# tennisonliu/bayesian-neural-network

Hardware: AMD Instinct MI355X
Metric: MC-forward-samples/sec + KL-elements/sec, 784-1200-1200-10 BNN (higher is better)
Workload: dtype bf16

## Files before the change

### bayesian-neural-network_amd/csrc/bbb_linear.hip

```cpp
#include "bnn_device.h"
#include "bnn_fin.h"
#include "bbb_sample_body.h"
#include "bbb_block_gemm.h"
#include "../../include/bnn_hip.h"
#include <string.h>

namespace bnn {

struct BbbK {
  const void* x;
  long x_sstride;
  const float* w_mu;
  const float* w_rho;
  const float* w_sigma;
  const float* b_mu;
  const float* b_rho;
  const float* eps_w;
  const float* eps_b;
  float* eps_w_dump;
  float* eps_b_dump;
  void* y;
  float4* ws;
  int S, B, K, N;
  __bf16* y16;
// ... 175 lines not shown
        bf16x4 o;
#pragma unroll
        for (int i = 0; i < 4; ++i) o[i] = (__bf16)v[i];
        *reinterpret_cast<bf16x4*>(yp) = o;
      } else {
#pragma unroll
        for (int i = 0; i < 4; ++i)
          if (nb + i < N) yp[i] = (__bf16)v[i];
      }
      if (p.y_lo) {
        __bf16* lp = reinterpret_cast<__bf16*>(p.y_lo) + yoff;
        bf16x4 l;
#pragma unroll
        for (int i = 0; i < 4; ++i) l[i] = (__bf16)(v[i] - (float)(__bf16)v[i]);
        if (vec_ok) {
          *reinterpret_cast<bf16x4*>(lp) = l;
        } else {
#pragma unroll
          for (int i = 0; i < 4; ++i)
            if (nb + i < N) lp[i] = l[i];
        }
      }
    } else {
      float* yp = reinterpret_cast<float*>(p.y) + yoff;
      if (vec_ok) {
        *reinterpret_cast<float4*>(yp) = make_float4(v[0], v[1], v[2], v[3]);
      } else {
#pragma unroll
        for (int i = 0; i < 4; ++i)
          if (nb + i < N) yp[i] = v[i];
      }
      if (p.y16) {
        __bf16* cp = p.y16 + yoff;
        if (vec_ok) {
          bf16x4 o;
#pragma unroll
          for (int i = 0; i < 4; ++i) o[i] = (__bf16)v[i];
          *reinterpret_cast<bf16x4*>(cp) = o;
        } else {
#pragma unroll
          for (int i = 0; i < 4; ++i)
            if (nb + i < N) cp[i] = (__bf16)v[i];
        }
      }
    }
  }
}

struct FinPack : FinTail {
  int ks;
  uint32_t* ks_ticket;
  float4* ks_stats;
  float* ks_tiles;
};

template <int MATH, int XDT, int R, bool ALIGNED, bool FINAL, bool TRANS = false, bool PRE = false, int MT = 8, bool WT = false,
          bool XTL = false>
__device__ __forceinline__ bool bbb_fwd_body(const BbbK& p, const FinPack* fp) {
  constexpr int F = 16 / R;
  static_assert(!XTL || (FINAL && R == 1 && ALIGNED && MT == 8 && XDT == BNN_BF16 && MATH == BNN_MATH_BF16),
                "piece-order x: the fused output layer in bf16 math");
  extern __shared__ __attribute__((aligned(16))) float lds[];
  const int lane = threadIdx.x & 63, wave = threadIdx.x >> 6, nw = blockDim.x >> 6;
  const int r = lane & 15, q = lane >> 4;
  const int c = r / F, f = r % F;
  const int K = p.K, N = p.N, B = p.B;
  const int ntiles = (N + F - 1) / F, mbs = (B + 16 * MT - 1) / (16 * MT);
  int item;
  const int KS = FINAL ? fp->ks : 1;
  if (!xcd_work_item(ntiles * p.S * mbs * KS, item)) return false;
  const int ks = item % KS;
  item /= KS;
  const int nt = item / (p.S * mbs), s = (item / mbs) % p.S, mb = item % mbs;
  const int n = nt * F + f;
  const bool n_ok = n < N;
  const int nc = min(n, N - 1);
  const int m0 = mb * (16 * MT);
  const int mtiles = min(MT, (B - m0 + 15) >> 4);
  const int ssteps = (K + 32 * R - 1) / (32 * R);
  const int spb = (ssteps + KS - 1) / KS;
  const int t_lo = ks * spb, t_hi = min(ssteps, t_lo + spb);
  const uint32_t gs = global_sample(p, s);
  const bool do_stats = p.want_stats && mb == 0;
  const bool do_ls = do_stats && (s == 0 || FINAL);
  const bool do_dump = mb == 0;
  const int gpr = (int)eps_groups_per_row(K);
  const uint32_t wid = eps_tensor_id(p.layer_id, kEpsWeight);
  const char* xs = reinterpret_cast<const char*>(p.x) + (size_t)(s / p.xg) * (size_t)p.x_sstride * (XDT == BNN_F32 ? 4 : 2);
  constexpr bool X3 = MATH == BNN_MATH_BF16X3;
  static_assert(!X3 || (!TRANS && !PRE && !WT), "the split-bf16 mode is a forward sampling form");
  const char* xs_lo = (X3 && XDT == BNN_BF16) ? reinterpret_cast<const char*>(p.x_lo) + (size_t)(s / p.xg) * (size_t)p.x_sstride * 2 : nullptr;

  float* lds_bias = lds + (size_t)nw * MT * 64 * 4;
  float* lds_red = lds_bias + 16;
  f32x4* slab = reinterpret_cast<f32x4*>(lds);

  BNN_STAMP(0);
  BNN_STAMP_RT(8);
  f32x4 acc[MT];
#pragma unroll
  for (int m = 0; m < MT; ++m) acc[m] = f32x4{0.f, 0.f, 0.f, 0.f};
  float s_e2 = 0.f, s_a = 0.f, s_ls = 0.f;
  if (do_stats && item == 0 && ks == 0 && threadIdx.x == 0)
    p.ws[0] = make_float4(__int_as_float(ntiles), 0.f, 0.f, 0.f);

  float mu_n[8], rho_n[8];
  float4 wraw_n = make_float4(0.f, 0.f, 0.f, 0.f);
  auto load_params = [&](int t) {
    const int k = (t * R + c) * 32 + q * 8;
    if (PRE && TRANS) {
      bf16x8 tw;
#pragma unroll
      for (int j = 0; j < 8; ++j) {
        const __bf16 v = p.w_pre[((size_t)s * K + min(k + j, K - 1)) * p.ldw + nc];
        tw[j] = (k + j < K && n_ok) ? v : (__bf16)0.f;
      }
      wraw_n = __builtin_bit_cast(float4, tw);
    } else if (PRE) {
      wraw_n = *reinterpret_cast<const float4*>(p.w_pre + ((size_t)s * N + nc) * K + min(k, K - 8));
    } else if (TRANS) {
#pragma unroll
      for (int j = 0; j < 8; ++j) {
        const size_t woff = (size_t)min(k + j, K - 1) * p.ldw + nc;
        mu_n[j] = p.w_mu[woff];
        rho_n[j] = p.w_rho[woff];
      }
    } else if (ALIGNED) {
      const size_t woff = (size_t)nc * K + min(k, K - 8);
      load8<true>(p.w_mu + woff, 8, mu_n);
      load8<true>(p.w_rho + woff, 8, rho_n);
    } else {
      const int valid = n_ok ? min(8, K - k) : 0;
      const size_t woff = (size_t)n * K + k;
      load8<false>(p.w_mu + woff, valid, mu_n);
      load8<false>(p.w_rho + woff, valid, rho_n);
    }
  };
  if (t_lo + wave < t_hi) load_params(t_lo + wave);
  float bmu_pre = 0.f, brho_pre = 0.f, beps_pre = 0.f;
  if (PRE) {
    if (!TRANS && wave == nw - 1 && lane < F && n_ok && ks == 0 && p.b_pre) bmu_pre = p.b_pre[(size_t)s * N + n];
  } else if (!TRANS && wave == nw - 1 && lane < F && n_ok && ks == 0) {
    bmu_pre = p.b_mu[n];
    brho_pre = p.b_rho[n];
    beps_pre = bias_eps(p, n, s, gs, do_dump);
  }

#pragma nounroll
  for (int t = t_lo + wave; t < t_hi; t += nw) {
    const int k = (t * R + c) * 32 + q * 8;
    const int valid = n_ok ? min(8, K - k) : 0;
    constexpr int FR = (XDT == BNN_F32 || X3) ? 2 : 1;
    constexpr int MC0 = (8 / (R * FR)) < 1 ? 1 : (8 / (R * FR));
    constexpr int MC = MC0 > MT ? MT : MC0;
    float4 xraw[MC * R * FR];
    auto stage = [&](int ch) {
#pragma unroll
      for (int mm = 0; mm < MC; ++mm) {
        if constexpr (XTL) {
          xraw[mm] = *reinterpret_cast<const float4*>(xs + ((size_t)((t * 8 + ch * MC + mm) * 64 + lane)) * 16);
          continue;
        }
        const int row = m0 + (ch * MC + mm) * 16 + r;
#pragma unroll
        for (int cc = 0; cc < R; ++cc) {
          const int xk = (t * R + cc) * 32 + q * 8;
          if (ALIGNED) {
            const size_t off = (size_t)min(row, B - 1) * K + min(xk, K - 8);
            if (XDT == BNN_F32) {
              const float4* px = reinterpret_cast<const float4*>(reinterpret_cast<const float*>(xs) + off);
              xraw[(mm * R + cc) * 2 + 0] = px[0];
              xraw[(mm * R + cc) * 2 + 1] = px[1];
            } else if (X3) {
              xraw[(mm * R + cc) * 2 + 0] = *reinterpret_cast<const float4*>(reinterpret_cast<const __bf16*>(xs) + off);
              xraw[(mm * R + cc) * 2 + 1] = *reinterpret_cast<const float4*>(reinterpret_cast<const __bf16*>(xs_lo) + off);
            } else {
              xraw[mm * R + cc] = *reinterpret_cast<const float4*>(reinterpret_cast<const __bf16*>(xs) + off);
            }
          } else {
            const int xvalid = (row < B) ? min(8, K - xk) : 0;
            const size_t off = (size_t)row * K + xk;
            if (XDT == BNN_F32) {
              float v[8];
              load8<false>(reinterpret_cast<const float*>(xs) + off, xvalid, v);
              xraw[(mm * R + cc) * 2 + 0] = make_float4(v[0], v[1], v[2], v[3]);
              xraw[(mm * R + cc) * 2 + 1] = make_float4(v[4], v[5], v[6], v[7]);
            } else {
              bf16x8 vb;
#pragma unroll
              for (int j = 0; j < 8; ++j)
                vb[j] = (j < xvalid) ? (reinterpret_cast<const __bf16*>(xs) + off)[j] : (__bf16)0.0f;
              if (X3) {
                bf16x8 vl;
#pragma unroll
                for (int j = 0; j < 8; ++j)
                  vl[j] = (j < xvalid) ? (reinterpret_cast<const __bf16*>(xs_lo) + off)[j] : (__bf16)0.0f;
                xraw[(mm * R + cc) * 2 + 0] = __builtin_bit_cast(float4, vb);
                xraw[(mm * R + cc) * 2 + 1] = __builtin_bit_cast(float4, vl);
              } else {
// ... 129 lines not shown
              bf16x8 xb;
              if (XDT == BNN_F32) {
                const float4 lo = xraw[(mm * R + cc) * 2], hi = xraw[(mm * R + cc) * 2 + 1];
                xb[0] = (__bf16)lo.x; xb[1] = (__bf16)lo.y; xb[2] = (__bf16)lo.z; xb[3] = (__bf16)lo.w;
                xb[4] = (__bf16)hi.x; xb[5] = (__bf16)hi.y; xb[6] = (__bf16)hi.z; xb[7] = (__bf16)hi.w;
              } else {
                xb = __builtin_bit_cast(bf16x8, xraw[mm * R + cc]);
              }
              acc[m] = __builtin_amdgcn_mfma_f32_16x16x32_bf16((R == 1 || c == cc) ? wa : wz, xb, acc[m], 0, 0, 0);
            } else {
              float xv[8];
              if (XDT == BNN_F32) {
                const float4 lo = xraw[(mm * R + cc) * 2], hi = xraw[(mm * R + cc) * 2 + 1];
                xv[0] = lo.x; xv[1] = lo.y; xv[2] = lo.z; xv[3] = lo.w;
                xv[4] = hi.x; xv[5] = hi.y; xv[6] = hi.z; xv[7] = hi.w;
              } else {
                const bf16x8 xb = __builtin_bit_cast(bf16x8, xraw[mm * R + cc]);
#pragma unroll
                for (int j = 0; j < 8; ++j) xv[j] = (float)xb[j];
              }
#pragma unroll
              for (int j = 0; j < 8; ++j)
                acc[m] = __builtin_amdgcn_mfma_f32_16x16x4f32((R == 1 || c == cc) ? w[j] : 0.f, xv[j], acc[m], 0, 0, 0);
            }
          }
        }
        if ((ch + 1) * MC < MT && (ch + 1) * MC < mtiles) stage(ch + 1);
      }
    }
  }

  asm volatile("" :: "v"(acc[0][0]), "v"(acc[MT - 1][3]));
  BNN_STAMP(3);
  if (wave == nw - 1 && lane < 16) {
    float b = 0.f;
    if (PRE) b = (!TRANS && lane < F && n_ok && ks == 0) ? bmu_pre : 0.f;
    else if (!TRANS && lane < F && n_ok && ks == 0) b = sample_bias(p, bmu_pre, brho_pre, beps_pre, do_stats, do_ls, s_e2, s_a, s_ls);
    lds_bias[lane] = b;
  }
#pragma unroll
  for (int m = 0; m < MT; ++m)
    if (m < mtiles) slab[(wave * MT + m) * 64 + lane] = acc[m];
  if (do_stats) {
    const float a = wave_sum(s_e2), b = wave_sum(s_a), cc = wave_sum(s_ls);
    if (lane == 0) {
      lds_red[wave * 3 + 0] = a;
      lds_red[wave * 3 + 1] = b;
      lds_red[wave * 3 + 2] = cc;
    }
  }
  BNN_STAMP(4);
  __syncthreads();
  BNN_STAMP(5);
  float own0 = 0.f, own1 = 0.f, own2 = 0.f;
  if (do_stats && threadIdx.x == 0) {
    for (int wv = 0; wv < nw; ++wv) {
      own0 += lds_red[wv * 3 + 0];
      own1 += lds_red[wv * 3 + 1];
      own2 += lds_red[wv * 3 + 2];
    }
    if (KS == 1) p.ws[1 + (size_t)s * ntiles + nt] = make_float4(own0, own1, own2, 0.f);
  }
  float* fin_lg = lds_red + 3 * nw;
  if (!FINAL || KS == 1) {
    epilogue_store<R, MT>(p, slab, lds_bias, nw, mtiles, nt, s, m0, FINAL ? fin_lg : nullptr);
  }
  BNN_STAMP(6);
  BNN_STAMP_RT(9);
  if (FINAL) {
    const FinK& fk = fp->k;
    float* part = reinterpret_cast<float*>((reinterpret_cast<uintptr_t>(fin_lg + 128 * 16) + 7) & ~(uintptr_t)7);
    int T[8];
#pragma unroll
    for (int l = 0; l < 8; ++l)
      T[l] = (l < fk.n_layers - 1) ? __float_as_int(reinterpret_cast<const float4*>(fk.ws[l])[0].x) : 0;
    if (KS > 1) {
      float* mine = fp->ks_tiles + ((size_t)s * KS + ks) * (128 * 16);
      epilogue_store<R>(p, slab, lds_bias, nw, 8, nt, s, m0, nullptr, mine);
      if (threadIdx.x == 0) fp->ks_stats[(size_t)s * KS + ks] = make_float4(own0, own1, own2, 0.f);
      asm volatile("s_waitcnt vmcnt(0)" ::: "memory");
      __syncthreads();
      uint32_t* flag = reinterpret_cast<uint32_t*>(part);
      if (threadIdx.x == 0) {
        __builtin_amdgcn_fence(__ATOMIC_RELEASE, "agent");
        asm volatile("s_waitcnt vmcnt(0)" ::: "memory");
        const uint32_t tk = __hip_atomic_fetch_add(fp->ks_ticket + s, 1u, __ATOMIC_RELAXED, __HIP_MEMORY_SCOPE_AGENT);
        const uint32_t last = (tk == (uint32_t)KS - 1u) ? 1u : 0u;
        if (last) {
          __builtin_amdgcn_fence(__ATOMIC_ACQUIRE, "agent");
          asm volatile("s_waitcnt vmcnt(0)" ::: "memory");
        }
        *flag = last;
      }
      __syncthreads();
      BNN_STAMP(7);
      if (*flag == 0u) return true;
      __syncthreads();
      const float* tiles = fp->ks_tiles + (size_t)s * KS * (128 * 16);
      float4 q4 = make_float4(0.f, 0.f, 0.f, 0.f);
      if ((int)threadIdx.x < KS) q4 = fp->ks_stats[(size_t)s * KS + threadIdx.x];
      for (int it = threadIdx.x; it < 128 * 4; it += blockDim.x) {
        const int brow = it >> 2, fg = it & 3;
        f32x4 v = f32x4{0.f, 0.f, 0.f, 0.f};
        for (int j = 0; j < KS; ++j) v += *reinterpret_cast<const f32x4*>(tiles + (size_t)j * (128 * 16) + brow * 16 + fg * 4);
        if (p.relu) {
#pragma unroll
          for (int i = 0; i < 4; ++i) v[i] = fmaxf(v[i], 0.f);
        }
        *reinterpret_cast<f32x4*>(fin_lg + brow * 16 + fg * 4) = v;
        if (brow < B) {
          float* yp = reinterpret_cast<float*>(p.y) + ((size_t)s * B + brow) * N + fg * 4;
#pragma unroll
          for (int i = 0; i < 4; ++i)
            if (fg * 4 + i < N) yp[i] = v[i];
        }
      }
      if (threadIdx.x < 64) {
        own0 = wave_sum(q4.x);
        own1 = wave_sum(q4.y);
        own2 = wave_sum(q4.z);
      }
      if (threadIdx.x == 0) {
        p.ws[1 + (size_t)s * ntiles + nt] = make_float4(own0, own1, own2, 0.f);
        fp->ks_ticket[s] = 0u;
      }
    }
    __syncthreads();
    BNN_STAMP(10);
    float a = 0.f, b = 0.f, nll = 0.f;
    const int own_layer = fk.n_layers - 1;
#ifdef BNN_STAMPS
    fin_sample(fk, fp->c, s, T, fin_lg, 16, own_layer, own0, own1, own2, part, a, b, nll, p.dbg ? p.dbg + (size_t)blockIdx.x * 16 : nullptr);
#else
    fin_sample(fk, fp->c, s, T, fin_lg, 16, own_layer, own0, own1, own2, part, a, b, nll);
#endif
    BNN_STAMP(11);
    if (threadIdx.x == 0) {
      fin_store(fk, s, a, b, nll);
      if (fk.S == 1) {
        if (fp->sums) {
          float* so = fp->sums;
          so[0] = a; so[1] = b; so[2] = nll; so[3] = 1.f;
        }
        if (fk.sample_counter) *fk.sample_counter += fk.sample_counter_inc;
      } else if (fp->ticket) {
        fin_samples_meet(fk, fp->sums, fp->ticket);
      }
    }
  }
  return true;
}

template <int MATH, int XDT, int R, bool ALIGNED>
__global__ __launch_bounds__(768) void bbb_fwd_kernel(const BbbK p) {
  bbb_fwd_body<MATH, XDT, R, ALIGNED, false>(p, nullptr);
}

template <int MATH, int XDT, bool XTL = false>
__global__ __launch_bounds__(768) void bbb_fwd_final_kernel(const BbbK p, const FinPack fp) {
  bbb_fwd_body<MATH, XDT, 1, true, true, false, false, 8, false, XTL>(p, &fp);
}

template <int XDT, int R>
__global__ __launch_bounds__(768) void bbb_fwd_rider_kernel(const BbbK p, const SampleK sk, int n_main) {
  if ((int)blockIdx.x >= n_main) {
    extern __shared__ __attribute__((aligned(16))) float lds[];
    sample_block(sk, (int)blockIdx.x - n_main, lds);
    return;
  }
  bbb_fwd_body<BNN_MATH_BF16, XDT, R, true, false>(p, nullptr);
}

struct FinRows {
  const void* x;
  long x_sstride;
  int xg;
  const __bf16* w;
  const float* b;
  float* y;
  int S, B, K, N, relu;
  uint32_t* tickets;
  float* parts;
};

template <bool XF32>
__global__ __launch_bounds__(256) void bbb_final_rows_kernel(const FinRows p, const FinPack fp, const FinLoss tr) {
  __shared__ __attribute__((aligned(16))) f32x4 red[4][64];
  __shared__ float lg[16][17];
  __shared__ __attribute__((aligned(8))) float part[4 * kFinNV];
  const FinK& fk = fp.k;
  const int RB = (p.B + 15) >> 4;
  const int s = (int)blockIdx.x / (RB + 1), rb = (int)blockIdx.x - s * (RB + 1);
  const int lane = threadIdx.x & 63, wave = threadIdx.x >> 6;
  float pub0 = 0.f, pub1 = 0.f;
  int slot = rb;
  if (rb == RB) {
    int T[8];
#pragma unroll
    for (int l = 0; l < 8; ++l) T[l] = (l < fk.n_layers) ? __float_as_int(reinterpret_cast<const float4*>(fk.ws[l])[0].x) : 0;
    float a = 0.f, b = 0.f, nll = 0.f;
    fin_sample(fk, fp.c, s, T, nullptr, 0, -1, 0.f, 0.f, 0.f, part, a, b, nll);
// ... 1474 lines not shown
  return BNN_OK;
}

extern "C" int bnn_bbb_linear_fwd(const bnn_bbb_fwd_args* a, void* stream_) {
  return bbb_linear_fwd_impl(a, stream_, false, nullptr, 0);
}

static constexpr int kFinalTicketMaxSamples = 16;
static constexpr int kRowsTicketMaxSamples = 64;

extern "C" size_t bnn_bbb_final_scratch_bytes(int32_t n_samples) {
  return n_samples <= 0 ? 0 : fin_scratch(nullptr, (size_t)n_samples).bytes;
}

extern "C" int bnn_bbb_final_fwd(const bnn_bbb_fwd_args* a, const bnn_finalize_args* f, void* stream_) {
  BbbK k;
  bool al = false;
  int rc = prepare(a, k, al);
  if (rc != BNN_OK) return rc;
  const bool x_pieces = a->x_layout == BNN_LAYOUT_PIECES;
  if (a->y_layout || a->w_pieces || (x_pieces && (a->w_sampled || a->math != BNN_MATH_BF16))) return BNN_ERR_ENUM;
  FinPack fp;
  rc = make_fin(f, fp.k, fp.c);
  if (rc != BNN_OK) return rc;
  const int nl = f->n_layers;
  rc = check_fin_loss(f);
  if (rc != BNN_OK) return rc;
  if (a->w_sampled) {
    const int S = a->n_samples, B = a->batch, N = a->out_features, K = a->in_features;
    const bool rows = a->y_dtype == BNN_F32 && N <= 16 && B <= 128 && S <= 4096 && !f->local_reparam &&
                      nl >= 1 && f->n_samples == S && f->classes == N && f->batch == B && f->logits == a->y && f->nll &&
                      f->scratch && f->scratch_bytes >= bnn_bbb_final_scratch_bytes(S) &&
                      !(reinterpret_cast<uintptr_t>(f->scratch) & 15) &&
                      (S == 1 || f->ticket || (S > kRowsTicketMaxSamples && !f->loss)) && !a->rider &&
                      (N % 4 != 0 || !(reinterpret_cast<uintptr_t>(a->y) & 15));
    if (!rows) {
      rc = bnn_bbb_linear_fwd(a, stream_);
      if (rc == BNN_OK) rc = bnn_elbo_finalize(f, stream_);
      return rc != BNN_OK ? rc : bnn_loss_tail_(f, stream_);
    }
    const FinLoss tr = make_fin_loss(f);
    FinRows fr;
    fr.x = a->x;
    fr.x_sstride = k.x_sstride; fr.xg = k.xg;
    fr.w = k.w_pre; fr.b = k.b_pre;
    fr.y = reinterpret_cast<float*>(a->y);
    fr.S = S; fr.B = B; fr.K = K; fr.N = N; fr.relu = a->relu ? 1 : 0;
    const FinScratch sc = fin_scratch(f->scratch, (size_t)S);
    fr.tickets = sc.tickets;
    fr.parts = sc.stats;
    const bool rows_tail = S > kRowsTicketMaxSamples && !tr.out4;
    fp.sums = f->sums;
    fp.ticket = rows_tail ? nullptr : f->ticket;
    fp.ks = 1; fp.ks_ticket = nullptr; fp.ks_stats = nullptr; fp.ks_tiles = nullptr;
    const int RB = (B + 15) / 16;
    if (a->x_dtype == BNN_BF16)
      hipLaunchKernelGGL(bbb_final_rows_kernel<false>, dim3((unsigned)(S * (RB + 1))), dim3(256), 0, reinterpret_cast<hipStream_t>(stream_),
                         fr, fp, tr);
    else
      hipLaunchKernelGGL(bbb_final_rows_kernel<true>, dim3((unsigned)(S * (RB + 1))), dim3(256), 0, reinterpret_cast<hipStream_t>(stream_),
                         fr, fp, tr);
    const hipError_t e2 = hipGetLastError();
    if (e2 != hipSuccess) return (int)e2;
    return rows_tail ? bnn_elbo_sums_(f, stream_) : (int)BNN_OK;
  }
  const bool fuse = al && a->out_features <= 16 && a->batch <= 128 && a->want_stats && !f->local_reparam && nl >= 1 &&
                    f->layer_workspace[nl - 1] == a->workspace && f->n_samples == a->n_samples &&
                    f->classes == a->out_features && f->batch == a->batch && a->y_dtype == BNN_F32 &&
                    (a->n_samples == 1 || a->n_samples > kFinalTicketMaxSamples || f->ticket != nullptr) && !(a->log_prior || a->log_q) &&
                    a->form == BNN_FORM_AUTO;
  if (x_pieces && !fuse) return BNN_ERR_ENUM;
  if (!fuse) {
    rc = bnn_bbb_linear_fwd(a, stream_);
    if (rc != BNN_OK) return rc;
    rc = bnn_elbo_finalize(f, stream_);
    return rc != BNN_OK ? rc : bnn_loss_tail_(f, stream_);
  }
  hipStream_t stream = reinterpret_cast<hipStream_t>(stream_);
  fp.sums = f->sums;
  const bool tail_kernel = a->n_samples > kFinalTicketMaxSamples;
  fp.ticket = tail_kernel ? nullptr : f->ticket;
  const int K = a->in_features;
  const int ssteps = (K + 31) / 32;
  if (x_pieces) k.x_sstride = a->x_per_sample ? (long)ssteps * 4096 : 0;
  int KS = (ssteps + 11) / 12;
  KS = KS > kFinalMaxSlices ? kFinalMaxSlices : KS;
  for (int ks = KS; ks <= kFinalMaxSlices; ++ks) {
    const int per = (ssteps + ks - 1) / ks;
    if (per <= 12 && ((per & 3) == 0 || per < 4)) {
      KS = ks;
      break;
    }
  }
  if ((long)a->n_samples * KS > 128) KS = 1;
  if (KS > 1 && (!f->scratch || f->scratch_bytes < bnn_bbb_final_scratch_bytes(a->n_samples) ||
                 (reinterpret_cast<uintptr_t>(f->scratch) & 15)))
    KS = 1;
  const int spb = (ssteps + KS - 1) / KS;
  int spw = 1;
  while ((spb + spw - 1) / spw > 12) ++spw;
  int nw = (spb + spw - 1) / spw;
  nw = nw < 1 ? 1 : nw;
  fp.ks = KS;
  const FinScratch sc = fin_scratch(f->scratch, (size_t)a->n_samples);
  fp.ks_ticket = sc.tickets;
  fp.ks_stats = reinterpret_cast<float4*>(sc.stats);
  fp.ks_tiles = sc.tiles;
  const long total = (long)a->n_samples * KS;
  hipError_t err = hipSuccess;
  const dim3 grid((unsigned)(((total + 7) / 8) * 8)), block(nw * 64);
  const size_t lds = ((size_t)nw * 8 * 64 * 4 + 16 + 3 * nw + 128 * 16 + kFinMaxWaves * kFinNV) * sizeof(float);
#define BNN_FIN(MATH, XDT)                                                                     \
  do {                                                                                         \
    err = allow_big_lds(bbb_fwd_final_kernel<MATH, XDT>, lds);                                 \
    if (err == hipSuccess)                                                                     \
      hipLaunchKernelGGL((bbb_fwd_final_kernel<MATH, XDT>), grid, block, lds, stream, k, fp);  \
  } while (0)
  if (x_pieces) {
    err = allow_big_lds(bbb_fwd_final_kernel<BNN_MATH_BF16, BNN_BF16, true>, lds);
    if (err == hipSuccess)
      hipLaunchKernelGGL((bbb_fwd_final_kernel<BNN_MATH_BF16, BNN_BF16, true>), grid, block, lds, stream, k, fp);
  } else if (a->math == BNN_MATH_BF16) {
    if (a->x_dtype == BNN_F32) BNN_FIN(BNN_MATH_BF16, BNN_F32); else BNN_FIN(BNN_MATH_BF16, BNN_BF16);
  } else if (a->math == BNN_MATH_BF16X3) {
    if (a->x_dtype == BNN_F32) BNN_FIN(BNN_MATH_BF16X3, BNN_F32); else BNN_FIN(BNN_MATH_BF16X3, BNN_BF16);
  } else {
    if (a->x_dtype == BNN_F32) BNN_FIN(BNN_MATH_F32, BNN_F32); else BNN_FIN(BNN_MATH_F32, BNN_BF16);
  }
#undef BNN_FIN
  if (err != hipSuccess) return (int)err;
  err = hipGetLastError();
  if (err != hipSuccess) return (int)err;
  rc = tail_kernel ? bnn_elbo_sums_(f, stream_) : (int)BNN_OK;
  return rc != BNN_OK ? rc : bnn_loss_tail_(f, stream_);
// ... 90 lines not shown
```

### bayesian-neural-network_amd/csrc/bnn_fin.h

```cpp
#pragma once
#include "bnn_device.h"
#include "bnn_prior.h"
#include "bnn_nll_row.h"
#include "../../include/bnn_hip.h"
#include <math.h>

extern "C" int bnn_elbo_sums_(const bnn_finalize_args* f, void* stream);
extern "C" int bnn_loss_tail_(const bnn_finalize_args* f, void* stream);

namespace bnn {

struct FinK {
  const float* ws[8];
  int lin[8], lout[8];
  int n_layers, local_reparam, S, B, C;
  bnn_prior prior;
  const float* logits;
  const void* target;
  int nll_mode;
  float nll_sigma;
  float *log_prior, *log_q, *kl, *nll;
  uint32_t* sample_counter;
  uint32_t sample_counter_inc;
  int group;
// ... 30 lines not shown
};
static inline FinScratch fin_scratch(void* base, size_t S) {
  const size_t tickets = ((S * 4 + 255) / 256) * 256, stats = S * kFinalMaxSlices * 16, tiles = S * kFinalMaxSlices * (128 * 16 * 4);
  const uintptr_t b = reinterpret_cast<uintptr_t>(base);
  return {reinterpret_cast<uint32_t*>(b), reinterpret_cast<float*>(b + tickets), reinterpret_cast<float*>(b + tickets + stats),
          tickets + stats + tiles};
}

static inline int make_fin(const bnn_finalize_args* a, FinK& k, FinC& cst) {
  if (!a) return BNN_ERR_NULL;
  if (a->struct_bytes != sizeof(bnn_finalize_args)) return BNN_ERR_ABI;
  if (a->n_layers < 0 || a->n_layers > 8 || a->n_samples <= 0 || a->n_samples > 65535) return BNN_ERR_SHAPE;
  if (prior_check(a->prior) == BNN_ERR_ENUM || (unsigned)a->nll_mode > 1u) return BNN_ERR_ENUM;
  for (int l = 0; l < 8; ++l) {
    k.ws[l] = l < a->n_layers ? reinterpret_cast<const float*>(a->layer_workspace[l]) : nullptr;
    k.lin[l] = l < a->n_layers ? a->layer_in[l] : 0;
    k.lout[l] = l < a->n_layers ? a->layer_out[l] : 0;
    if (l < a->n_layers) {
      if (!k.ws[l]) return BNN_ERR_NULL;
      if (reinterpret_cast<uintptr_t>(k.ws[l]) & 15) return BNN_ERR_ALIGN;
      if (k.lin[l] <= 0 || k.lout[l] <= 0) return BNN_ERR_SHAPE;
    }
  }
  if (a->n_layers > 0 && a->prior.kind != BNN_PRIOR_MIXTURE && prior_check(a->prior) != BNN_OK) return BNN_ERR_SHAPE;
  if (a->group_samples < 0 || (a->group_samples > 0 && a->n_samples % a->group_samples != 0)) return BNN_ERR_SHAPE;
  if (a->target_per_group && a->group_samples <= 0) return BNN_ERR_SHAPE;
  if (a->nll) {
    if (!a->logits || !a->target) return BNN_ERR_NULL;
    if (a->batch <= 0 || a->classes <= 0) return BNN_ERR_SHAPE;
    if (a->nll_mode == BNN_NLL_REGRESSION && !(a->nll_sigma > 0.f)) return BNN_ERR_SHAPE;
  }
  k.n_layers = a->n_layers; k.local_reparam = a->local_reparam; k.S = a->n_samples; k.B = a->batch; k.C = a->classes;
  k.prior = a->prior; k.logits = a->logits; k.target = a->target; k.nll_mode = a->nll_mode;
  k.nll_sigma = a->nll_sigma; k.log_prior = a->log_prior; k.log_q = a->log_q; k.kl = a->kl; k.nll = a->nll;
  k.sample_counter = a->sample_counter; k.sample_counter_inc = a->sample_counter_inc;
  k.group = a->group_samples;
  k.nll_partial = nullptr; k.nll_rb = 0;
  k.tgt_stride = a->target_per_group
                     ? (a->nll_mode == BNN_NLL_CLASSIFICATION ? (long)a->batch : (long)a->batch * a->classes) : 0;
  for (int l = 0; l < 8; ++l) cst.cnt_c0[l] = cst.lp_const[l] = cst.kl_const[l] = 0.0;
  for (int l = 0; l < a->n_layers; ++l) {
    const PriorFold f = prior_fold_make(a->prior, (double)a->layer_out[l] * a->layer_in[l] + a->layer_out[l]);
    cst.cnt_c0[l] = f.cnt_c0;
    cst.lp_const[l] = f.lp_const;
    cst.kl_const[l] = f.kl_const;
  }
  cst.inv2var = prior_fold_make(a->prior, 0.0).inv2var;
  const double ns = a->nll_sigma > 0.f ? (double)a->nll_sigma : 1.0;
  cst.reg_const = log(ns) - kNegLogSqrt2Pi;
  cst.reg_inv2var = 1.0 / (2.0 * ns * ns);
  return BNN_OK;
}

__device__ __forceinline__ float fin_nll(const FinK& p, const FinC& cst, int s, const float* lg, int ldc, int row0, int row1) {
  const int lane = threadIdx.x & 63, wave = threadIdx.x >> 6;
  float acc = 0.f;
    if (p.nll_mode == BNN_NLL_CLASSIFICATION) {
    const long long* tgt = reinterpret_cast<const long long*>(p.target) + (p.group > 0 ? (s / p.group) * p.tgt_stride : 0);
    if (p.C <= 32) {
      for (int b = row0 + (int)threadIdx.x; b < row1; b += blockDim.x) {
        const float* row = lg + (size_t)b * ldc;
        const long long tc = tgt[b];
        float mx, se = 0.f;
        if (ldc == 16 && p.C <= 16) {
          float vr[16];
#pragma unroll
          for (int i = 0; i < 16; ++i) vr[i] = row[(i + b) & 15];
          mx = -3.0e38f;
#pragma unroll
          for (int i = 0; i < 16; ++i) mx = (((i + b) & 15) < p.C) ? fmaxf(mx, vr[i]) : mx;
#pragma unroll
          for (int i = 0; i < 16; ++i) se += (((i + b) & 15) < p.C) ? __expf(vr[i] - mx) : 0.f;
          se = __logf(se);
        } else if (p.C <= 16) {
          float vr[16];
#pragma unroll
          for (int i = 0; i < 16; ++i) vr[i] = row[min(i, p.C - 1)];
          mx = vr[0];
#pragma unroll
          for (int i = 1; i < 16; ++i) mx = i < p.C ? fmaxf(mx, vr[i]) : mx;
#pragma unroll
          for (int i = 0; i < 16; ++i) se += i < p.C ? __expf(vr[i] - mx) : 0.f;
          se = __logf(se);
        } else {
          mx = row[0];
          for (int cc = 1; cc < p.C; ++cc) mx = fmaxf(mx, row[cc]);
          for (int cc = 0; cc < p.C; ++cc) se += expf(row[cc] - mx);
          se = logf(se);
        }
        const float picked = (tc >= 0 && tc < p.C) ? row[tc] : __builtin_nanf("");
        acc += (mx + se) - picked;
      }
    } else {
      const int nwv = blockDim.x >> 6;
      for (int b = row0 + wave; b < row1; b += nwv) {
        const float* row = lg + (size_t)b * ldc;
        float mx = -3.0e38f;
#pragma unroll 8
        for (int cc = lane; cc < p.C; cc += 64) mx = fmaxf(mx, row[cc]);
#pragma unroll
        for (int off = 32; off > 0; off >>= 1) mx = fmaxf(mx, __shfl_xor(mx, off, 64));
        float se = 0.f;
#pragma unroll 8
        for (int cc = lane; cc < p.C; cc += 64) se += __expf(row[cc] - mx);
        se = wave_sum(se);
        if (lane == 0) {
          const long long tc = tgt[b];
          const float picked = (tc >= 0 && tc < p.C) ? row[tc] : __builtin_nanf("");
          acc += (mx + logf(se)) - picked;
        }
      }
    }
  } else {
    const float* tgt = reinterpret_cast<const float*>(p.target) + (p.group > 0 ? (s / p.group) * p.tgt_stride : 0);
    if (p.C <= 8) {
      for (int b = row0 + (int)threadIdx.x; b < row1; b += blockDim.x)
        for (int cc = 0; cc < p.C; ++cc) {
          const float d = tgt[(size_t)b * p.C + cc] - lg[(size_t)b * ldc + cc];
          acc += (float)((double)(d * d) * cst.reg_inv2var + cst.reg_const);
        }
    } else {
      const int nwv = blockDim.x >> 6;
      float d2 = 0.f;
      int cnt = 0;
      for (int b = row0 + wave; b < row1; b += nwv) {
        const float* row = lg + (size_t)b * ldc;
        const float* trow = tgt + (size_t)b * p.C;
        if (((p.C | ldc) & 3) == 0 && ((reinterpret_cast<uintptr_t>(row) | reinterpret_cast<uintptr_t>(trow)) & 15) == 0) {
#pragma unroll 4
          for (int cc = lane * 4; cc < p.C; cc += 256) {
            const float4 t4 = *reinterpret_cast<const float4*>(trow + cc), r4 = *reinterpret_cast<const float4*>(row + cc);
            const float dx = t4.x - r4.x, dy = t4.y - r4.y, dz = t4.z - r4.z, dw = t4.w - r4.w;
            d2 = __builtin_fmaf(dx, dx, __builtin_fmaf(dy, dy, __builtin_fmaf(dz, dz, __builtin_fmaf(dw, dw, d2))));
            cnt += 4;
          }
        } else {
#pragma unroll 8
          for (int cc = lane; cc < p.C; cc += 64) {
            const float d = trow[cc] - row[cc];
            d2 = __builtin_fmaf(d, d, d2);
            ++cnt;
          }
        }
      }
      acc = (float)((double)d2 * cst.reg_inv2var + (double)cnt * cst.reg_const);
    }
  }
  return acc;
}

__device__ __forceinline__ float fin_row_nll(const FinK& fk, const FinC& cst, int s, int brow, const float* lgrow) {
  const int C = fk.C;
  float acc_n = 0.f;
  if (fk.nll_mode == BNN_NLL_CLASSIFICATION) {
    const long long* tgt = reinterpret_cast<const long long*>(fk.target) + (fk.group > 0 ? (s / fk.group) * fk.tgt_stride : 0);
    const long long tc = tgt[brow];
    float mx = -3.0e38f, se = 0.f;
    for (int c = 0; c < C; ++c) mx = fmaxf(mx, lgrow[c]);
    for (int c = 0; c < C; ++c) se += __expf(lgrow[c] - mx);
    const float picked = (tc >= 0 && tc < C) ? lgrow[(int)tc] : __builtin_nanf("");
    acc_n = (mx + __logf(se)) - picked;
  } else {
    const float* tgt = reinterpret_cast<const float*>(fk.target) + (fk.group > 0 ? (s / fk.group) * fk.tgt_stride : 0);
    for (int c = 0; c < C; ++c) {
      const float d = tgt[(size_t)brow * C + c] - lgrow[c];
      acc_n += (float)((double)(d * d) * cst.reg_inv2var + cst.reg_const);
    }
  }
  return acc_n;
}

__device__ __forceinline__ void fin_sample(const FinK& p, const FinC& cst, int s, const int T[8], const float* lg, int ldc,
                                           int own_layer, float own0, float own1, float own2, float* part,
                                           float& out_a, float& out_b, float& out_nll, unsigned long long* dbg = nullptr) {
#define FIN_STAMP(i) do { if (dbg && threadIdx.x == 0) dbg[i] = __builtin_amdgcn_s_memtime(); } while (0)
  constexpr int NV = kFinNV;
  const int lane = threadIdx.x & 63, wave = threadIdx.x >> 6;
  float v[NV];
#pragma unroll
  for (int i = 0; i < NV; ++i) v[i] = 0.f;
#pragma unroll
  for (int l = 0; l < 8; ++l) {
    if (l < p.n_layers && l != own_layer) {
      const float4* ws = reinterpret_cast<const float4*>(p.ws[l]);
      const int Tl = T[l], bd = blockDim.x;
      constexpr int FU = 8;
      for (int t0 = threadIdx.x; t0 < Tl; t0 += FU * bd) {
        float4 qv[FU];
        float lsz[FU];
#pragma unroll
        for (int u = 0; u < FU; ++u) {
          const int t = min(t0 + u * bd, Tl - 1);
          qv[u] = p.local_reparam ? ws[1 + t] : ws[1 + (size_t)s * Tl + t];
          lsz[u] = p.local_reparam ? 0.f : ws[1 + t].z;
        }
#pragma unroll
        for (int u = 0; u < FU; ++u) {
          if (t0 + u * bd < Tl) {
            v[3 * l + 0] += qv[u].x;
            v[3 * l + 1] += qv[u].y;
            v[3 * l + 2] += p.local_reparam ? qv[u].z : lsz[u];
          }
        }
      }
    }
  }
  FIN_STAMP(12);
  if (p.nll && p.nll_partial) {
    float acc = 0.f;
    for (int t = threadIdx.x; t < p.nll_rb; t += blockDim.x) acc += p.nll_partial[(size_t)s * p.nll_rb + t];
    v[NV - 1] = acc;
  } else if (p.nll && lg) {
    v[NV - 1] = fin_nll(p, cst, s, lg, ldc, 0, p.B);
  }
  FIN_STAMP(13);
  const int nv = 3 * p.n_layers;
  if (nv <= 9) {
    float t[10];
#pragma unroll
    for (int i = 0; i < 9; ++i) t[i] = wave_sum(v[i]);
    t[9] = wave_sum(v[NV - 1]);
    if (lane == 0) {
#pragma unroll
      for (int i = 0; i < 9; ++i) part[wave * NV + i] = t[i];
      part[wave * NV + NV - 1] = t[9];
    }
  } else {
#pragma unroll
    for (int i = 0; i < NV; ++i) {
      if (i < nv || i == NV - 1) {
        const float t = wave_sum(v[i]);
        if (lane == 0) part[wave * NV + i] = t;
      }
    }
  }
  FIN_STAMP(14);
  __syncthreads();
  double folded = 0;
  {
    const int nwv = blockDim.x >> 6;
    if ((int)threadIdx.x < NV && ((int)threadIdx.x < nv || (int)threadIdx.x == NV - 1))
      for (int w = 0; w < nwv; ++w) folded += (double)part[w * NV + threadIdx.x];
  }
  __syncthreads();
  if ((int)threadIdx.x < NV) reinterpret_cast<double*>(part)[threadIdx.x] = folded;
  __syncthreads();
  FIN_STAMP(15);
  if (threadIdx.x == 0) {
    auto red = [&](int i) { return reinterpret_cast<const double*>(part)[i]; };
    float a_tot = 0.f, b_tot = 0.f;
#pragma unroll
    for (int l = 0; l < 8; ++l) {
      if (l >= p.n_layers) break;
      double r0, r1, r2;
      if (l == own_layer) {
        r0 = own0; r1 = own1; r2 = own2;
      } else {
        r0 = red(3 * l); r1 = red(3 * l + 1); r2 = red(3 * l + 2);
      }
      if (p.local_reparam) {
        a_tot += (float)(cst.kl_const[l] - r0 + (r1 + r2) * cst.inv2var);
      } else {
        const double lq = fold_log_q(cst.cnt_c0[l], r2, r0);
        const double lp = fold_log_p(p.prior.kind, cst.lp_const[l], cst.inv2var, r1);
        a_tot += (float)lp;
        b_tot += (float)lq;
// ... 49 lines not shown
  const int g = p.group > 0 ? p.group : p.S;
  const float* pa = p.local_reparam ? p.kl : p.log_prior;
  const float* pb = (!p.local_reparam && p.log_q) ? p.log_q : nullptr;
  fin_fold_groups(pa, pb, p.nll, p.S, g, [&](int m, double ta, double tb, double tn) {
    float* so = sums + 4 * m;
    so[0] = (float)ta; so[1] = (float)tb; so[2] = (float)tn; so[3] = (float)g;
  });
}

__device__ __forceinline__ void fin_store(const FinK& p, int s, float a, float b, float nll) {
  if (p.local_reparam) {
    if (p.kl) p.kl[s] = a;
  } else {
    if (p.log_prior) p.log_prior[s] = a;
    if (p.log_q) p.log_q[s] = b;
  }
  if (p.nll) p.nll[s] = nll;
}

struct FinLoss {
  const float* beta;
  float total, grad_scale, inv_var;
  float* out4;
  float* g_a;
  float* g_b;
  float* g_kl3;
  float* g_logits;
};

__device__ __forceinline__ void fin_loss_assemble(const FinK& fk, const FinLoss& tr) {
  const float* pa = fk.local_reparam ? fk.kl : fk.log_prior;
  double x = 0, y = 0, z = 0;
  fin_fold_groups(pa, fk.local_reparam ? nullptr : fk.log_q, fk.nll, fk.S, fk.S, [&](int, double ta, double tb, double tn) { x = ta; y = tb; z = tn; });
  const float beta = *tr.beta;
  const float inv = tr.grad_scale / tr.total;
  for (int i = 0; i < fk.S; ++i) {
    if (tr.g_a) tr.g_a[i] = fk.local_reparam ? 0.f : -beta * inv;
    if (tr.g_b) tr.g_b[i] = beta * inv;
  }
  const float am = (float)x / tr.total, bm = (float)y / tr.total, nm = (float)z / tr.total;
  tr.out4[0] = fk.local_reparam ? beta * am + nm : beta * bm - beta * am + nm;
  tr.out4[1] = am;
  tr.out4[2] = bm;
  tr.out4[3] = nm;
  if (tr.g_kl3) { tr.g_kl3[0] = beta * tr.grad_scale; tr.g_kl3[1] = 0.f; tr.g_kl3[2] = 0.f; }
}

__device__ __forceinline__ void fin_loss_row_grad(const FinK& fk, const FinLoss& tr, int s, int B, int brow, const float* lgrow) {
  nll_row_grad(lgrow, fk.C, fk.nll_mode, fk.target, brow, tr.grad_scale / tr.total, tr.inv_var,
               tr.g_logits + ((size_t)s * B + brow) * fk.C);
}


template <int NSTAT>
__device__ __forceinline__ void fin_rows_meet(const FinK& fk, const FinLoss& tr, float* sums, uint32_t* ticket, uint32_t* tickets, float* parts,
                                              int s, int slot, float pub0, float pub1, int RB, int last) {
  static_assert(NSTAT == 1 || NSTAT == 2, "KL | log p, log q");
  float* mine = parts + (size_t)s * 16;
  __hip_atomic_store(mine + slot, pub0, __ATOMIC_RELAXED, __HIP_MEMORY_SCOPE_AGENT);
  if (NSTAT == 2 && slot == 8) __hip_atomic_store(mine + 9, pub1, __ATOMIC_RELAXED, __HIP_MEMORY_SCOPE_AGENT);
  asm volatile("s_waitcnt vmcnt(0)" ::: "memory");
  const uint32_t tk = __hip_atomic_fetch_add(tickets + s, 1u, __ATOMIC_RELAXED, __HIP_MEMORY_SCOPE_AGENT);
  if (tk != (uint32_t)last) return;
  float pv[8 + NSTAT];
#pragma unroll
  for (int i = 0; i < 8 + NSTAT; ++i) pv[i] = __hip_atomic_load(mine + i, __ATOMIC_RELAXED, __HIP_MEMORY_SCOPE_AGENT);
  double tn = 0;
#pragma unroll
  for (int i = 0; i < 8; ++i)
    if (i < RB) tn += pv[i];
  const float a = pv[8], b = NSTAT == 2 ? pv[8 + NSTAT - 1] : 0.f;
  const float nll = (float)tn;
  __hip_atomic_store(tickets + s, 0u, __ATOMIC_RELAXED, __HIP_MEMORY_SCOPE_AGENT);
  float* const out_a = NSTAT == 2 ? fk.log_prior : fk.kl;
  if (out_a) __hip_atomic_store(out_a + s, a, __ATOMIC_RELAXED, __HIP_MEMORY_SCOPE_AGENT);
  if (NSTAT == 2 && fk.log_q) __hip_atomic_store(fk.log_q + s, b, __ATOMIC_RELAXED, __HIP_MEMORY_SCOPE_AGENT);
  if (fk.nll) __hip_atomic_store(fk.nll + s, nll, __ATOMIC_RELAXED, __HIP_MEMORY_SCOPE_AGENT);
  if (fk.S == 1) {
    if (sums) {
      sums[0] = a; sums[1] = b; sums[2] = nll; sums[3] = 1.f;
    }
    if (tr.out4) fin_loss_assemble(fk, tr);
    if (fk.sample_counter) *fk.sample_counter += fk.sample_counter_inc;
    return;
  }
  if (!ticket) return;
  asm volatile("s_waitcnt vmcnt(0)" ::: "memory");
  const uint32_t t2 = __hip_atomic_fetch_add(ticket, 1u, __ATOMIC_RELAXED, __HIP_MEMORY_SCOPE_AGENT);
  if (t2 != (uint32_t)fk.S - 1u) return;
  if (sums) fin_fold_sums(fk, sums);
  if (tr.out4) fin_loss_assemble(fk, tr);
  __hip_atomic_store(ticket, 0u, __ATOMIC_RELAXED, __HIP_MEMORY_SCOPE_AGENT);
  if (fk.sample_counter) *fk.sample_counter += fk.sample_counter_inc;
}

__device__ __forceinline__ void fin_samples_meet(const FinK& fk, float* sums, uint32_t* ticket) {
  __builtin_amdgcn_fence(__ATOMIC_RELEASE, "agent");
  asm volatile("s_waitcnt vmcnt(0)" ::: "memory");
  const uint32_t tk = __hip_atomic_fetch_add(ticket, 1u, __ATOMIC_RELAXED, __HIP_MEMORY_SCOPE_AGENT);
  if (tk != (uint32_t)fk.S - 1u) return;
  __builtin_amdgcn_fence(__ATOMIC_ACQUIRE, "agent");
  asm volatile("s_waitcnt vmcnt(0)" ::: "memory");
  if (sums) fin_fold_sums(fk, sums);
  *ticket = 0u;
  if (fk.sample_counter) *fk.sample_counter += fk.sample_counter_inc;
}
// ... 23 lines not shown
```

Before: 526,500.

## Prefetch final-layer KL stats and targets early; add group1 ticket path

```diff
diff --git a/bayesian-neural-network_amd/csrc/bbb_linear.hip b/bayesian-neural-network_amd/csrc/bbb_linear.hip
--- a/bayesian-neural-network_amd/csrc/bbb_linear.hip
+++ b/bayesian-neural-network_amd/csrc/bbb_linear.hip
@@ -251,7 +251,12 @@
   uint32_t* ks_ticket;
   float4* ks_stats;
   float* ks_tiles;
+  int group1;
 };
+
+#ifndef BNN_K1C_TAIL_PARTS
+#define BNN_K1C_TAIL_PARTS 3
+#endif
 
 template <int MATH, int XDT, int R, bool ALIGNED, bool FINAL, bool TRANS = false, bool PRE = false, int MT = 8, bool WT = false,
           bool XTL = false>
@@ -280,6 +285,15 @@
   const int spb = (ssteps + KS - 1) / KS;
   const int t_lo = ks * spb, t_hi = min(ssteps, t_lo + spb);
   const uint32_t gs = global_sample(p, s);
+  constexpr bool FIN_EARLY = FINAL && MATH == BNN_MATH_BF16 && XDT == BNN_BF16 && (BNN_K1C_TAIL_PARTS & 2) != 0;
+  int fin_T[8];
+  FinPre fin_pre{};
+  if constexpr (FIN_EARLY) {
+#pragma unroll
+    for (int l = 0; l < 8; ++l)
+      fin_T[l] = (l < fp->k.n_layers - 1)
+                     ? __builtin_amdgcn_readfirstlane(__float_as_int(reinterpret_cast<const float4*>(fp->k.ws[l])[0].x)) : 0;
+  }
   const bool do_stats = p.want_stats && mb == 0;
   const bool do_ls = do_stats && (s == 0 || FINAL);
   const bool do_dump = mb == 0;
@@ -344,6 +358,7 @@
     brho_pre = p.b_rho[n];
     beps_pre = bias_eps(p, n, s, gs, do_dump);
   }
+  if constexpr (FIN_EARLY) fin_pre = fin_preload(fp->k, s, fin_T, fp->k.n_layers - 1);
 
 #pragma nounroll
   for (int t = t_lo + wave; t < t_hi; t += nw) {
@@ -579,6 +594,7 @@
   BNN_STAMP(4);
   __syncthreads();
   BNN_STAMP(5);
+  if (FINAL && KS == 1 && fp->group1 && threadIdx.x == blockDim.x - 64) fin_group1_meet(fp->k, fp->ticket);
   float own0 = 0.f, own1 = 0.f, own2 = 0.f;
   if (do_stats && threadIdx.x == 0) {
     for (int wv = 0; wv < nw; ++wv) {
@@ -599,8 +615,10 @@
     float* part = reinterpret_cast<float*>((reinterpret_cast<uintptr_t>(fin_lg + 128 * 16) + 7) & ~(uintptr_t)7);
     int T[8];
 #pragma unroll
-    for (int l = 0; l < 8; ++l)
-      T[l] = (l < fk.n_layers - 1) ? __float_as_int(reinterpret_cast<const float4*>(fk.ws[l])[0].x) : 0;
+    for (int l = 0; l < 8; ++l) {
+      if constexpr (FIN_EARLY) T[l] = fin_T[l];
+      else T[l] = (l < fk.n_layers - 1) ? __float_as_int(reinterpret_cast<const float4*>(fk.ws[l])[0].x) : 0;
+    }
     if (KS > 1) {
       float* mine = fp->ks_tiles + ((size_t)s * KS + ks) * (128 * 16);
       epilogue_store<R>(p, slab, lds_bias, nw, 8, nt, s, m0, nullptr, mine);
@@ -656,10 +674,11 @@
     BNN_STAMP(10);
     float a = 0.f, b = 0.f, nll = 0.f;
     const int own_layer = fk.n_layers - 1;
+    const FinPre* pre = FIN_EARLY ? &fin_pre : nullptr;
 #ifdef BNN_STAMPS
-    fin_sample(fk, fp->c, s, T, fin_lg, 16, own_layer, own0, own1, own2, part, a, b, nll, p.dbg ? p.dbg + (size_t)blockIdx.x * 16 : nullptr);
+    fin_sample(fk, fp->c, s, T, fin_lg, 16, own_layer, own0, own1, own2, part, a, b, nll, p.dbg ? p.dbg + (size_t)blockIdx.x * 16 : nullptr, pre);
 #else
-    fin_sample(fk, fp->c, s, T, fin_lg, 16, own_layer, own0, own1, own2, part, a, b, nll);
+    fin_sample(fk, fp->c, s, T, fin_lg, 16, own_layer, own0, own1, own2, part, a, b, nll, nullptr, pre);
 #endif
     BNN_STAMP(11);
     if (threadIdx.x == 0) {
@@ -670,10 +689,13 @@
           so[0] = a; so[1] = b; so[2] = nll; so[3] = 1.f;
         }
         if (fk.sample_counter) *fk.sample_counter += fk.sample_counter_inc;
+      } else if (fp->group1) {
+        fin_group1_sums(fk, fp->sums, s, a, b, nll);
       } else if (fp->ticket) {
         fin_samples_meet(fk, fp->sums, fp->ticket);
       }
     }
+    if (KS > 1 && fp->group1 && threadIdx.x == blockDim.x - 64) fin_group1_meet(fk, fp->ticket);
   }
   return true;
 }
@@ -2254,7 +2276,7 @@
     const bool rows_tail = S > kRowsTicketMaxSamples && !tr.out4;
     fp.sums = f->sums;
     fp.ticket = rows_tail ? nullptr : f->ticket;
-    fp.ks = 1; fp.ks_ticket = nullptr; fp.ks_stats = nullptr; fp.ks_tiles = nullptr;
+    fp.ks = 1; fp.ks_ticket = nullptr; fp.ks_stats = nullptr; fp.ks_tiles = nullptr; fp.group1 = 0;
     const int RB = (B + 15) / 16;
     if (a->x_dtype == BNN_BF16)
       hipLaunchKernelGGL(bbb_final_rows_kernel<false>, dim3((unsigned)(S * (RB + 1))), dim3(256), 0, reinterpret_cast<hipStream_t>(stream_),
@@ -2280,8 +2302,11 @@
   }
   hipStream_t stream = reinterpret_cast<hipStream_t>(stream_);
   fp.sums = f->sums;
-  const bool tail_kernel = a->n_samples > kFinalTicketMaxSamples;
+  const bool many = a->n_samples > kFinalTicketMaxSamples;
+  const bool group1 = (BNN_K1C_TAIL_PARTS & 1) != 0 && many && f->group_samples == 1 && f->ticket != nullptr;
+  const bool tail_kernel = many && !group1;
   fp.ticket = tail_kernel ? nullptr : f->ticket;
+  fp.group1 = group1 ? 1 : 0;
   const int K = a->in_features;
   const int ssteps = (K + 31) / 32;
   if (x_pieces) k.x_sstride = a->x_per_sample ? (long)ssteps * 4096 : 0;
diff --git a/bayesian-neural-network_amd/csrc/bnn_fin.h b/bayesian-neural-network_amd/csrc/bnn_fin.h
--- a/bayesian-neural-network_amd/csrc/bnn_fin.h
+++ b/bayesian-neural-network_amd/csrc/bnn_fin.h
@@ -106,15 +106,52 @@
   return BNN_OK;
 }
 
-__device__ __forceinline__ float fin_nll(const FinK& p, const FinC& cst, int s, const float* lg, int ldc, int row0, int row1) {
+constexpr int kFinPreLayers = 2;
+struct FinPre {
+  float e2[kFinPreLayers], a[kFinPreLayers], ls[kFinPreLayers];
+  long long label;
+  float tval;
+  bool stats, row;
+};
+
+__device__ __forceinline__ FinPre fin_preload(const FinK& p, int s, const int T[8], int own_layer) {
+  FinPre pre;
+  pre.stats = !p.local_reparam && own_layer == p.n_layers - 1 && own_layer <= kFinPreLayers;
+#pragma unroll
+  for (int l = 0; l < kFinPreLayers; ++l)
+    if (l < own_layer) pre.stats = pre.stats && T[l] >= 1 && T[l] <= (int)blockDim.x;
+#pragma unroll
+  for (int l = 0; l < kFinPreLayers; ++l) {
+    const bool on = pre.stats && l < own_layer;
+    const float4* ws = reinterpret_cast<const float4*>(p.ws[min(l, p.n_layers - 1)]);
+    const int t = on ? min((int)threadIdx.x, T[l] - 1) : 0;
+    const float2 q = *reinterpret_cast<const float2*>(ws + 1 + (on ? (size_t)s * T[l] : (size_t)0) + t);
+    pre.e2[l] = q.x;
+    pre.a[l] = q.y;
+    pre.ls[l] = ws[1 + t].z;
+  }
+  pre.row = p.nll && !p.nll_partial && p.B >= 1 && p.B <= (int)blockDim.x &&
+            (p.nll_mode == BNN_NLL_CLASSIFICATION ? p.C <= 32 : p.C == 1);
+  const int b = min((int)threadIdx.x, p.B - 1);
+  const long goff = p.group > 0 ? (s / p.group) * p.tgt_stride : 0;
+  const void* standin = p.ws[0] + 4;
+  const bool cls = p.nll_mode == BNN_NLL_CLASSIFICATION;
+  pre.label = *((pre.row && cls) ? reinterpret_cast<const long long*>(p.target) + goff + b : reinterpret_cast<const long long*>(standin));
+  pre.tval = *((pre.row && !cls) ? reinterpret_cast<const float*>(p.target) + goff + b : reinterpret_cast<const float*>(standin));
+  return pre;
+}
+
+__device__ __forceinline__ float fin_nll(const FinK& p, const FinC& cst, int s, const float* lg, int ldc, int row0, int row1,
+                                         const FinPre* pre = nullptr) {
   const int lane = threadIdx.x & 63, wave = threadIdx.x >> 6;
+  const bool pre_row = pre && pre->row && row0 == 0;
   float acc = 0.f;
     if (p.nll_mode == BNN_NLL_CLASSIFICATION) {
     const long long* tgt = reinterpret_cast<const long long*>(p.target) + (p.group > 0 ? (s / p.group) * p.tgt_stride : 0);
     if (p.C <= 32) {
       for (int b = row0 + (int)threadIdx.x; b < row1; b += blockDim.x) {
         const float* row = lg + (size_t)b * ldc;
-        const long long tc = tgt[b];
+        const long long tc = pre_row ? pre->label : tgt[b];
         float mx, se = 0.f;
         if (ldc == 16 && p.C <= 16) {
           float vr[16];
@@ -170,7 +207,8 @@
     if (p.C <= 8) {
       for (int b = row0 + (int)threadIdx.x; b < row1; b += blockDim.x)
         for (int cc = 0; cc < p.C; ++cc) {
-          const float d = tgt[(size_t)b * p.C + cc] - lg[(size_t)b * ldc + cc];
+          const float tv = pre_row ? pre->tval : tgt[(size_t)b * p.C + cc];
+          const float d = tv - lg[(size_t)b * ldc + cc];
           acc += (float)((double)(d * d) * cst.reg_inv2var + cst.reg_const);
         }
     } else {
@@ -226,7 +264,8 @@
 
 __device__ __forceinline__ void fin_sample(const FinK& p, const FinC& cst, int s, const int T[8], const float* lg, int ldc,
                                            int own_layer, float own0, float own1, float own2, float* part,
-                                           float& out_a, float& out_b, float& out_nll, unsigned long long* dbg = nullptr) {
+                                           float& out_a, float& out_b, float& out_nll, unsigned long long* dbg = nullptr,
+                                           const FinPre* pre = nullptr) {
 #define FIN_STAMP(i) do { if (dbg && threadIdx.x == 0) dbg[i] = __builtin_amdgcn_s_memtime(); } while (0)
   constexpr int NV = kFinNV;
   const int lane = threadIdx.x & 63, wave = threadIdx.x >> 6;
@@ -236,6 +275,14 @@
 #pragma unroll
   for (int l = 0; l < 8; ++l) {
     if (l < p.n_layers && l != own_layer) {
+      if (pre && pre->stats) {
+        if (l < kFinPreLayers && (int)threadIdx.x < T[l]) {
+          v[3 * l + 0] += pre->e2[l < kFinPreLayers ? l : 0];
+          v[3 * l + 1] += pre->a[l < kFinPreLayers ? l : 0];
+          v[3 * l + 2] += pre->ls[l < kFinPreLayers ? l : 0];
+        }
+        continue;
+      }
       const float4* ws = reinterpret_cast<const float4*>(p.ws[l]);
       const int Tl = T[l], bd = blockDim.x;
       constexpr int FU = 8;
@@ -265,7 +312,7 @@
     for (int t = threadIdx.x; t < p.nll_rb; t += blockDim.x) acc += p.nll_partial[(size_t)s * p.nll_rb + t];
     v[NV - 1] = acc;
   } else if (p.nll && lg) {
-    v[NV - 1] = fin_nll(p, cst, s, lg, ldc, 0, p.B);
+    v[NV - 1] = fin_nll(p, cst, s, lg, ldc, 0, p.B, pre);
   }
   FIN_STAMP(13);
   const int nv = 3 * p.n_layers;
@@ -421,6 +468,23 @@
 }
 
 
+__device__ __forceinline__ void fin_group1_sums(const FinK& fk, float* sums, int s, float a, float b, float nll) {
+  if (!sums) return;
+  const bool has_a = fk.local_reparam ? fk.kl != nullptr : fk.log_prior != nullptr;
+  const bool has_b = !fk.local_reparam && fk.log_q != nullptr;
+  float* so = sums + 4 * (size_t)s;
+  so[0] = has_a ? (float)(0.0 + (double)a) : 0.f;
+  so[1] = has_b ? (float)(0.0 + (double)b) : 0.f;
+  so[2] = fk.nll ? (float)(0.0 + (double)nll) : 0.f;
+  so[3] = 1.f;
+}
+__device__ __forceinline__ void fin_group1_meet(const FinK& fk, uint32_t* ticket) {
+  const uint32_t tk = __hip_atomic_fetch_add(ticket, 1u, __ATOMIC_RELAXED, __HIP_MEMORY_SCOPE_AGENT);
+  if (tk != (uint32_t)fk.S - 1u) return;
+  __hip_atomic_store(ticket, 0u, __ATOMIC_RELAXED, __HIP_MEMORY_SCOPE_AGENT);
+  if (fk.sample_counter) *fk.sample_counter += fk.sample_counter_inc;
+}
+
 template <int NSTAT>
 __device__ __forceinline__ void fin_rows_meet(const FinK& fk, const FinLoss& tr, float* sums, uint32_t* ticket, uint32_t* tickets, float* parts,
                                               int s, int slot, float pub0, float pub1, int RB, int last) {
```

New measurement: 530,700, median of 6. No clear change (+0.8%).
